# codelion/adaptive-classifier

Measured on NVIDIA H100. Metric: queries/sec predict() bert-base 128-tok, 1M x 768 prototypes, higher is better.
Workload: dtype f16

## Files before the change

### adaptive_classifier_b200/csrc/common.cuh

```cuda
#pragma once

#include <cuda_runtime.h>
#include <cuda.h>
#include <stdint.h>
#include <stdio.h>
#include <string.h>
#include <string>

#include "../../include/adaptive_b200.h"

namespace ac {

void set_error(const char *fmt, ...);
int check_cuda(cudaError_t e, const char *what);

#define AC_CUDA(call)                                                \
    do {                                                             \
        int _rc = ::ac::check_cuda((call), #call);                   \
        if (_rc != 0) return _rc;                                    \
    } while (0)

#define AC_REQUIRE(cond, ...)                                        \
    do {                                                             \
        if (!(cond)) {                                               \
// ... 58 lines not shown
    uint32_t ok;
    asm volatile(
        "{\n\t"
        ".reg .pred p;\n\t"
        "mbarrier.try_wait.parity.shared::cta.b64 p, [%1], %2;\n\t"
        "selp.u32 %0, 1, 0, p;\n\t"
        "}"
        : "=r"(ok)
        : "r"(smem_u32(bar)), "r"(parity)
        : "memory");
    return ok != 0;
}
__device__ __forceinline__ void mbar_wait(uint64_t *bar, uint32_t parity) {
    while (!mbar_try_wait(bar, parity)) {
    }
}

__device__ __forceinline__ void tma_prefetch_desc(const CUtensorMap *m) {
    asm volatile("prefetch.tensormap [%0];" ::"l"(reinterpret_cast<uint64_t>(m)) : "memory");
}
__device__ __forceinline__ void tma_load_2d(void *smem_dst, const CUtensorMap *m, uint64_t *bar, int c0, int c1) {
    asm volatile(
        "cp.async.bulk.tensor.2d.shared::cluster.global.tile.mbarrier::complete_tx::bytes [%0], [%1, {%3, %4}], [%2];"
        ::"r"(smem_u32(smem_dst)), "l"(reinterpret_cast<uint64_t>(m)), "r"(smem_u32(bar)), "r"(c0), "r"(c1)
        : "memory");
}
__device__ __forceinline__ void fence_proxy_async_smem() {
    asm volatile("fence.proxy.async.shared::cta;" ::: "memory");
}

__device__ __forceinline__ void named_bar_sync(int id, int nthreads) {
    asm volatile("bar.sync %0, %1;" ::"r"(id), "r"(nthreads) : "memory");
}

__device__ __forceinline__ uint64_t wgmma_desc_sw128(uint32_t smem_addr) {
    uint64_t d = 0;
    d |= static_cast<uint64_t>((smem_addr & 0x3FFFFu) >> 4);
    d |= static_cast<uint64_t>(1) << 16;
    d |= static_cast<uint64_t>(1024 >> 4) << 32;
    d |= static_cast<uint64_t>(1) << 62;
    return d;
}
__device__ __forceinline__ void wgmma_fence() { asm volatile("wgmma.fence.sync.aligned;" ::: "memory"); }
__device__ __forceinline__ void wgmma_commit() { asm volatile("wgmma.commit_group.sync.aligned;" ::: "memory"); }
template <int N>
__device__ __forceinline__ void wgmma_wait() { asm volatile("wgmma.wait_group.sync.aligned %0;" ::"n"(N) : "memory"); }

__device__ __forceinline__ void wgmma_m64n128_f16(float (&d)[64], uint64_t a_desc, uint64_t b_desc, uint32_t accumulate) {
    asm volatile(
        "{\n\t"
        ".reg .pred p;\n\t"
        "setp.ne.b32 p, %66, 0;\n\t"
        "wgmma.mma_async.sync.aligned.m64n128k16.f32.f16.f16 "
        "{%0, %1, %2, %3, %4, %5, %6, %7, %8, %9, %10, %11, %12, %13, %14, %15, "
        "%16, %17, %18, %19, %20, %21, %22, %23, %24, %25, %26, %27, %28, %29, %30, %31, "
        "%32, %33, %34, %35, %36, %37, %38, %39, %40, %41, %42, %43, %44, %45, %46, %47, "
        "%48, %49, %50, %51, %52, %53, %54, %55, %56, %57, %58, %59, %60, %61, %62, %63}, "
        "%64, %65, p, 1, 1, 0, 0;\n\t"
        "}"
        : "+f"(d[0]), "+f"(d[1]), "+f"(d[2]), "+f"(d[3]), "+f"(d[4]), "+f"(d[5]), "+f"(d[6]), "+f"(d[7]),
          "+f"(d[8]), "+f"(d[9]), "+f"(d[10]), "+f"(d[11]), "+f"(d[12]), "+f"(d[13]), "+f"(d[14]), "+f"(d[15]),
          "+f"(d[16]), "+f"(d[17]), "+f"(d[18]), "+f"(d[19]), "+f"(d[20]), "+f"(d[21]), "+f"(d[22]), "+f"(d[23]),
          "+f"(d[24]), "+f"(d[25]), "+f"(d[26]), "+f"(d[27]), "+f"(d[28]), "+f"(d[29]), "+f"(d[30]), "+f"(d[31]),
          "+f"(d[32]), "+f"(d[33]), "+f"(d[34]), "+f"(d[35]), "+f"(d[36]), "+f"(d[37]), "+f"(d[38]), "+f"(d[39]),
          "+f"(d[40]), "+f"(d[41]), "+f"(d[42]), "+f"(d[43]), "+f"(d[44]), "+f"(d[45]), "+f"(d[46]), "+f"(d[47]),
          "+f"(d[48]), "+f"(d[49]), "+f"(d[50]), "+f"(d[51]), "+f"(d[52]), "+f"(d[53]), "+f"(d[54]), "+f"(d[55]),
          "+f"(d[56]), "+f"(d[57]), "+f"(d[58]), "+f"(d[59]), "+f"(d[60]), "+f"(d[61]), "+f"(d[62]), "+f"(d[63])
// ... 77 lines not shown
```

### adaptive_classifier_b200/csrc/encoder.cu

```cuda
#include "gemm_tc.cuh"
#include <cuda_fp16.h>
#include <math_constants.h>
#include <algorithm>
#include <vector>

namespace ac {

__device__ __forceinline__ float ex2_approx(float x) {
    float y;
    asm("ex2.approx.ftz.f32 %0, %1;" : "=f"(y) : "f"(x));
    return y;
}
__device__ __forceinline__ float rcp_approx(float x) {
    float y;
    asm("rcp.approx.ftz.f32 %0, %1;" : "=f"(y) : "f"(x));
    return y;
}
__device__ __forceinline__ float gelu_erf(float y) {
    const float ay = fabsf(y);
    const float t = rcp_approx(fmaf(0.3275911f * 0.70710678118654752440f, ay, 1.f));
    float p = fmaf(0.5f * 1.061405429f, t, 0.5f * -1.453152027f);
    p = fmaf(p, t, 0.5f * 1.421413741f);
    p = fmaf(p, t, 0.5f * -0.284496736f);
    p = fmaf(p, t, 0.5f * 0.254829592f);
    const float e = ex2_approx((y * y) * (-0.5f * 1.4426950408889634f));
    const float h = (p * t) * e;
    return fmaxf(y, 0.f) - fabsf(y * h);
}

template <int MODE, bool OUT_HALF, bool VT, bool DEFER = false, bool ROPE = false>
struct EpiLinear {
    static_assert(!DEFER || (OUT_HALF && MODE != 2), "the deferred-LayerNorm consumer epilogues write fp16 operands");
    static_assert((MODE != 3 && !ROPE) || OUT_HALF, "the GeGLU / RoPE epilogues write fp16 operands");
    const float *__restrict__ bias;
    const float *__restrict__ residual;
    void *Y;
    int M, N, ldy;
    int round_out;
    __half *vT;
    int vt_col0, S, S_pad, H;
    const float *__restrict__ c1;
    const float2 *__restrict__ row_stats;
    const float *__restrict__ rope;

    static constexpr int kUnrollChunks = 4;
    static constexpr int kPrefetchDist = 1;
    struct State {
        float4 res[(MODE == 2) ? 2 : 1][(MODE == 2) ? 8 : 1];
        float mu, r;
    };
    __device__ __forceinline__ float pre(const State &st, float acc, float b, float c1v) const {
        return DEFER ? fmaf(st.r, fmaf(-st.mu, c1v, acc), b) : acc + b;
    }
    __device__ __forceinline__ bool skip_kernel() const { return false; }
    __device__ __forceinline__ void begin_cta(State &, int, int) const {}
    __device__ __forceinline__ void end_cta(State &, int, int) const {}

    __device__ __forceinline__ float act(float y) const {
        if (MODE == 1) y = gelu_erf(y);
        return y;
    }

    __device__ __forceinline__ void prefetch(State &st, const GemmTileInfo &ti, int row, int col0, int lane, int buf) const {
        if (DEFER) {
            if (((col0 - ti.n0) & (GEMM_EPI_COLS - 1)) == 0) {
                const float2 ms = (row < M) ? __ldg(row_stats + row) : make_float2(0.f, 0.f);
                st.mu = ms.x;
                st.r = ms.y;
            }
        }
        if (MODE != 2) return;
        const int row_base = row - lane;
        const int r8 = lane >> 2, c = lane & 3;
#pragma unroll
        for (int half = 0; half < 2; ++half) {
            const int col = col0 + 16 * half + 4 * c;
#pragma unroll
            for (int i = 0; i < 4; ++i) {
                const int grow = row_base + r8 + 8 * i;
                st.res[buf][half * 4 + i] =
                    (grow < M && col + 4 <= N)
                        ? __ldg(reinterpret_cast<const float4 *>(residual + static_cast<int64_t>(grow) * ldy + col))
                        : make_float4(0, 0, 0, 0);
            }
        }
    }

    __device__ __forceinline__ void tile(State &st, const GemmTileInfo &ti, int row, int col0, const float (&v)[32],
                                         uint8_t *stage, int lane, int buf, const float *acc) const {
// ... 103 lines not shown
                        const float4 a = *reinterpret_cast<const float4 *>(stage + rr * GEMM_EPI_STAGE_ROW_BYTES + 16 * c);
                        float4 o;
                        o.x = act(a.x + b4.x); o.y = act(a.y + b4.y); o.z = act(a.z + b4.z); o.w = act(a.w + b4.w);
                        if (MODE == 2) {
                            const float4 rs = st.res[buf][half * 4 + i];
                            o.x += rs.x; o.y += rs.y; o.z += rs.z; o.w += rs.w;
                        }
                        if (round_out) { o.x = round_tf32(o.x); o.y = round_tf32(o.y); o.z = round_tf32(o.z); o.w = round_tf32(o.w); }
                        *reinterpret_cast<float4 *>(Yf + static_cast<int64_t>(grow) * ldy + col) = o;
                    }
                }
                __syncwarp();
            }
        }
    }
};

struct EpiResidDefer {
    const float *__restrict__ bias;
    float *y;
    __half *yh;
    const float2 *__restrict__ stats_prev;
    const float *__restrict__ gamma;
    const float *__restrict__ beta;
    float2 *parts;
    int64_t part_stride;
    int M, N, ld;

    static constexpr int kUnrollChunks = 4;
#ifndef AC_RESID_PREFETCH
#define AC_RESID_PREFETCH 1
#endif
    static constexpr int kPrefetchDist = AC_RESID_PREFETCH;
    struct State {
        float4 res[kPrefetchDist + 1][8];
        float2 ms[4];
        float sum[4], sq[4];
    };
    __device__ __forceinline__ bool skip_kernel() const { return false; }
    __device__ __forceinline__ void begin_cta(State &, int, int) const {}
    __device__ __forceinline__ void end_cta(State &, int, int) const {}

    __device__ __forceinline__ void prefetch(State &st, const GemmTileInfo &ti, int row, int col0, int lane, int buf) const {
        const int row_base = row - lane;
        const int r8 = lane >> 2, c = lane & 3;
        if (((col0 - ti.n0) & (GEMM_EPI_COLS - 1)) == 0) {
#pragma unroll
            for (int i = 0; i < 4; ++i) {
                const int grow = row_base + r8 + 8 * i;
                st.ms[i] = (grow < M) ? __ldg(stats_prev + grow) : make_float2(0.f, 0.f);
                st.sum[i] = 0.f;
                st.sq[i] = 0.f;
            }
        }
#pragma unroll
        for (int half = 0; half < 2; ++half) {
            const int col = col0 + 16 * half + 4 * c;
#pragma unroll
            for (int i = 0; i < 4; ++i) {
                const int grow = row_base + r8 + 8 * i;
                st.res[buf][half * 4 + i] = (grow < M && col + 4 <= N)
                                                ? *reinterpret_cast<const float4 *>(y + static_cast<int64_t>(grow) * ld + col)
                                                : make_float4(0, 0, 0, 0);
            }
        }
    }

    __device__ __forceinline__ void tile(State &st, const GemmTileInfo &ti, int row, int col0, const float (&v)[32], uint8_t *stage,
                                         int lane, int buf, const float *) const {
        const int row_base = row - lane;
        if (row_base >= M || col0 >= N) return;
        const int r8 = lane >> 2, c = lane & 3;
#pragma unroll
        for (int half = 0; half < 2; ++half) {
            const int col = col0 + 16 * half + 4 * c;
            float4 *srow = reinterpret_cast<float4 *>(stage + lane * GEMM_EPI_STAGE_ROW_BYTES);
#pragma unroll
            for (int j = 0; j < 4; ++j)
                srow[j] = make_float4(v[16 * half + 4 * j], v[16 * half + 4 * j + 1], v[16 * half + 4 * j + 2], v[16 * half + 4 * j + 3]);
            __syncwarp();
            const bool col_ok = col + 4 <= N;
            const float4 b4 = col_ok ? __ldg(reinterpret_cast<const float4 *>(bias + col)) : make_float4(0, 0, 0, 0);
            const float4 g4 = col_ok ? __ldg(reinterpret_cast<const float4 *>(gamma + col)) : make_float4(0, 0, 0, 0);
            const float4 e4 = col_ok ? __ldg(reinterpret_cast<const float4 *>(beta + col)) : make_float4(0, 0, 0, 0);
#pragma unroll
            for (int i = 0; i < 4; ++i) {
                const int rr = r8 + 8 * i;
                const int grow = row_base + rr;
                if (grow < M && col_ok) {
                    const float4 a = *reinterpret_cast<const float4 *>(stage + rr * GEMM_EPI_STAGE_ROW_BYTES + 16 * c);
                    const float4 rs = st.res[buf][half * 4 + i];
                    const float mu = st.ms[i].x, r = st.ms[i].y;
                    float4 o;
                    o.x = (a.x + b4.x) + fmaf((rs.x - mu) * r, g4.x, e4.x);
                    o.y = (a.y + b4.y) + fmaf((rs.y - mu) * r, g4.y, e4.y);
                    o.z = (a.z + b4.z) + fmaf((rs.z - mu) * r, g4.z, e4.z);
                    o.w = (a.w + b4.w) + fmaf((rs.w - mu) * r, g4.w, e4.w);
                    *reinterpret_cast<float4 *>(y + static_cast<int64_t>(grow) * ld + col) = o;
                    const __half2 h0 = __floats2half2_rn(o.x, o.y), h1 = __floats2half2_rn(o.z, o.w);
                    uint2 pk;
                    pk.x = *reinterpret_cast<const uint32_t *>(&h0);
                    pk.y = *reinterpret_cast<const uint32_t *>(&h1);
                    *reinterpret_cast<uint2 *>(yh + static_cast<int64_t>(grow) * ld + col) = pk;
                    st.sum[i] += (o.x + o.y) + (o.z + o.w);
                    st.sq[i] += (o.x * o.x + o.y * o.y) + (o.z * o.z + o.w * o.w);
                }
            }
            __syncwarp();
        }
        if (((col0 - ti.n0) & (GEMM_EPI_COLS - 1)) == GEMM_EPI_COLS - 32) {
            const int part = col0 / GEMM_EPI_COLS;
#pragma unroll
            for (int i = 0; i < 4; ++i) {
                float s = st.sum[i], q = st.sq[i];
                s += __shfl_xor_sync(0xffffffffu, s, 1);
                q += __shfl_xor_sync(0xffffffffu, q, 1);
                s += __shfl_xor_sync(0xffffffffu, s, 2);
                q += __shfl_xor_sync(0xffffffffu, q, 2);
                const int grow = row_base + r8 + 8 * i;
                if (c == 0 && grow < M) parts[static_cast<int64_t>(part) * part_stride + grow] = make_float2(s, q);
            }
        }
    }
};

// ... 1064 lines not shown
```

### adaptive_classifier_b200/csrc/gemm_tc.cuh

```cuda
#pragma once
#include "common.cuh"

namespace ac {

constexpr int GEMM_BLOCK_M = 128;
constexpr int GEMM_BLOCK_N = 128;
constexpr int GEMM_BLOCK_K = 32;
constexpr int GEMM_KIND_TF32 = 0, GEMM_KIND_F16 = 1;
__host__ __device__ constexpr int gemm_block_k(int kind) { return kind == GEMM_KIND_F16 ? 64 : 32; }
constexpr int GEMM_STAGES = 4;
constexpr int GEMM_EPI_COLS = GEMM_BLOCK_N / 2;
constexpr int GEMM_EPI_WARPS = 8;
constexpr int GEMM_PRODUCER_THREAD = 32 * GEMM_EPI_WARPS;
constexpr int GEMM_THREADS = 32 * GEMM_EPI_WARPS + 128;
constexpr int GEMM_A_STAGE_BYTES = GEMM_BLOCK_M * 128;
constexpr int GEMM_B_STAGE_BYTES = GEMM_BLOCK_N * 128;
constexpr int GEMM_STAGE_BYTES = GEMM_A_STAGE_BYTES + GEMM_B_STAGE_BYTES;
constexpr int GEMM_ACC_LD = GEMM_BLOCK_N + 4;
constexpr int GEMM_ACC_BYTES = GEMM_BLOCK_M * GEMM_ACC_LD * 4;
constexpr int GEMM_EPI_STAGE_ROW_BYTES = 80;
constexpr int GEMM_EPI_STAGE_BYTES = 32 * GEMM_EPI_STAGE_ROW_BYTES;
constexpr int GEMM_SMEM_BYTES = GEMM_STAGES * GEMM_STAGE_BYTES + GEMM_ACC_BYTES + GEMM_EPI_WARPS * GEMM_EPI_STAGE_BYTES +
                                1024  + 256 ;
static_assert(GEMM_SMEM_BYTES <= 227 * 1024, "stage ring + accumulator tile do not fit");

#ifndef AC_MBAR_WATCHDOG
#define AC_MBAR_WATCHDOG 1
#endif

__device__ __forceinline__ void mbar_wait_guarded(uint64_t *bar, uint32_t parity) {
#if AC_MBAR_WATCHDOG
    uint32_t spins = 0;
    while (!mbar_try_wait(bar, parity)) {
        if (++spins > (1u << 26)) __trap();
    }
#else
    mbar_wait(bar, parity);
#endif
}

struct GemmTileInfo {
    int m0, n0;
    int tile_iter;
};

__device__ __forceinline__ int gemm_epi_chalf() { return ((threadIdx.x >> 5) >> 1) & 1; }

template <class Epi, bool kMFastest = false, int kKind = GEMM_KIND_TF32>
__global__ void __launch_bounds__(GEMM_THREADS, 1)
gemm_tc_kernel(const __grid_constant__ CUtensorMap tmap_a, const __grid_constant__ CUtensorMap tmap_b,
               int M, int N, int K, Epi epi) {
    if (epi.skip_kernel()) return;
    extern __shared__ uint8_t smem_raw[];
    uint8_t *smem = reinterpret_cast<uint8_t *>((reinterpret_cast<uintptr_t>(smem_raw) + 1023) & ~uintptr_t(1023));
    uint8_t *smem_a = smem;
    uint8_t *smem_b = smem + GEMM_STAGES * GEMM_A_STAGE_BYTES;
    float *acc_tile = reinterpret_cast<float *>(smem + GEMM_STAGES * GEMM_STAGE_BYTES);
    uint8_t *epi_stage = smem + GEMM_STAGES * GEMM_STAGE_BYTES + GEMM_ACC_BYTES;
    uint64_t *bars = reinterpret_cast<uint64_t *>(epi_stage + GEMM_EPI_WARPS * GEMM_EPI_STAGE_BYTES);
    uint64_t *full_bar = bars;
    uint64_t *empty_bar = bars + GEMM_STAGES;

    const int warp = threadIdx.x >> 5;
    const int lane = threadIdx.x & 31;
    const int tiles_m = (M + GEMM_BLOCK_M - 1) / GEMM_BLOCK_M;
    const int tiles_n = (N + GEMM_BLOCK_N - 1) / GEMM_BLOCK_N;
    const int num_tiles = tiles_m * tiles_n;
    constexpr int BK = gemm_block_k(kKind);
    const int num_kb = (K + BK - 1) / BK;

    if (threadIdx.x == GEMM_PRODUCER_THREAD) {
        tma_prefetch_desc(&tmap_a);
        tma_prefetch_desc(&tmap_b);
        for (int s = 0; s < GEMM_STAGES; ++s) {
            mbar_init(&full_bar[s], 1);
            mbar_init(&empty_bar[s], GEMM_EPI_WARPS);
        }
        fence_mbar_init();
    }
    __syncthreads();

    if (threadIdx.x >= GEMM_PRODUCER_THREAD) {
        if (threadIdx.x == GEMM_PRODUCER_THREAD) {
            int stage = 0;
            uint32_t phase = 0;
            for (int tile = blockIdx.x; tile < num_tiles; tile += gridDim.x) {
                const int m0 = (kMFastest ? tile % tiles_m : tile / tiles_n) * GEMM_BLOCK_M;
                const int n0 = (kMFastest ? tile / tiles_m : tile % tiles_n) * GEMM_BLOCK_N;
                for (int kb = 0; kb < num_kb; ++kb) {
                    mbar_wait_guarded(&empty_bar[stage], phase ^ 1);
                    mbar_arrive_expect_tx(&full_bar[stage], GEMM_STAGE_BYTES);
                    tma_load_2d(smem_a + stage * GEMM_A_STAGE_BYTES, &tmap_a, &full_bar[stage], kb * BK, m0);
                    tma_load_2d(smem_b + stage * GEMM_B_STAGE_BYTES, &tmap_b, &full_bar[stage], kb * BK, n0);
                    if (++stage == GEMM_STAGES) { stage = 0; phase ^= 1; }
                }
            }
        }
        return;
    }

    const int wg = warp >> 2;
    const int q = 2 * wg + (warp & 1);
    const int chalf = gemm_epi_chalf();
    typename Epi::State est;
    epi.begin_cta(est, q, lane);
    int stage = 0;
    uint32_t phase = 0;
    int it = 0;
    const float *acc_row = acc_tile + (q * 32 + lane) * GEMM_ACC_LD;
    for (int tile = blockIdx.x; tile < num_tiles; tile += gridDim.x, ++it) {
        GemmTileInfo ti;
        ti.m0 = (kMFastest ? tile % tiles_m : tile / tiles_n) * GEMM_BLOCK_M;
        ti.n0 = (kMFastest ? tile / tiles_m : tile % tiles_n) * GEMM_BLOCK_N;
        ti.tile_iter = it;
        const int row = ti.m0 + q * 32 + lane;
        const int c_lo = chalf * GEMM_EPI_COLS;
        constexpr int kDist = Epi::kPrefetchDist, kBufs = kDist + 1, kChunks = GEMM_EPI_COLS / 32;
#pragma unroll
        for (int d = 0; d < kDist; ++d)
            if (d < kChunks) epi.prefetch(est, ti, row, ti.n0 + c_lo + 32 * d, lane, d % kBufs);

        float acc[64];
#pragma unroll
        for (int j = 0; j < 64; ++j) acc[j] = 0.f;
        int prev_stage = -1;
        for (int kb = 0; kb < num_kb; ++kb) {
            mbar_wait_guarded(&full_bar[stage], phase);
            const uint64_t a_desc = wgmma_desc_sw128(smem_u32(smem_a + stage * GEMM_A_STAGE_BYTES + wg * 64 * 128));
            const uint64_t b_desc = wgmma_desc_sw128(smem_u32(smem_b + stage * GEMM_B_STAGE_BYTES));
            wgmma_fence();
#pragma unroll
            for (int k = 0; k < 4; ++k) {
                if (kKind == GEMM_KIND_F16) wgmma_m64n128_f16(acc, a_desc + 2 * k, b_desc + 2 * k, 1u);
                else wgmma_m64n128_tf32(acc, a_desc + 2 * k, b_desc + 2 * k, 1u);
            }
            wgmma_commit();
            wgmma_wait<1>();
            __syncwarp();
            if (prev_stage >= 0 && lane == 0) mbar_arrive(&empty_bar[prev_stage]);
            prev_stage = stage;
            if (++stage == GEMM_STAGES) { stage = 0; phase ^= 1; }
        }
        wgmma_wait<0>();
        __syncwarp();
        if (lane == 0) mbar_arrive(&empty_bar[prev_stage]);

        named_bar_sync(1 + wg, 128);
        wgmma_store_acc(acc, acc_tile + wg * 64 * GEMM_ACC_LD, GEMM_ACC_LD);
        named_bar_sync(1 + wg, 128);
#pragma unroll (Epi::kUnrollChunks)
        for (int ci = 0; ci < kChunks; ++ci) {
            const int c = c_lo + 32 * ci;
            if (ci + kDist < kChunks) epi.prefetch(est, ti, row, ti.n0 + c + 32 * kDist, lane, (ci + kDist) % kBufs);
            float v[32];
            acc_row_ld32(acc_row + c, v);
            epi.tile(est, ti, row, ti.n0 + c, v, epi_stage + warp * GEMM_EPI_STAGE_BYTES, lane, ci % kBufs, acc_row + c);
        }
    }
    epi.end_cta(est, q, lane);
}

template <class Epi, bool kMFastest = false, int kKind = GEMM_KIND_TF32>
int launch_gemm_tc(const CUtensorMap &ta, const CUtensorMap &tb, int M, int N, int K, const Epi &epi,
                   cudaStream_t stream, int max_ctas = 0, int prof_cls = PROF_GEMM_LINEAR, double prof_bytes = 0.0) {
    auto kern = gemm_tc_kernel<Epi, kMFastest, kKind>;
    static bool attr_set[64] = {};
    int dev = 0;
    AC_CUDA(cudaGetDevice(&dev));
    if (dev < 0 || dev >= 64 || !attr_set[dev]) {
        AC_CUDA(cudaFuncSetAttribute(kern, cudaFuncAttributeMaxDynamicSharedMemorySize, GEMM_SMEM_BYTES));
        if (dev >= 0 && dev < 64) attr_set[dev] = true;
    }
    const int tiles = ((M + GEMM_BLOCK_M - 1) / GEMM_BLOCK_M) * ((N + GEMM_BLOCK_N - 1) / GEMM_BLOCK_N);
    int ctas = sm_count();
    if (max_ctas > 0 && max_ctas < ctas) ctas = max_ctas;
    if (tiles < ctas) ctas = tiles;
    if (ctas <= 0) return AC_OK;
    const int slot = prof_begin(prof_cls, 2.0 * M * static_cast<double>(N) * K, prof_bytes, stream);
    kern<<<ctas, GEMM_THREADS, GEMM_SMEM_BYTES, stream>>>(ta, tb, M, N, K, epi);
    prof_end(slot, stream);
    AC_LAUNCH_CHECK();
    return AC_OK;
}

}
```

### adaptive_classifier_b200/csrc/knn_tc.cu

```cuda
#include "gemm_tc.cuh"
#include <cuda_fp16.h>
#include <math_constants.h>

namespace ac {

int launch_knn_rerank(const float *Q, const float *P, int B, int64_t N, int D, int kc, const int32_t *cand, float *out_d,
                      int64_t *out_i, int64_t row_offset, cudaStream_t stream);
size_t topk_select_workspace(int B, int64_t L, int k);
int topk_select(const float *d, const int64_t *idx, int B, int64_t L, int64_t in_stride, int64_t id_offset, int k,
                float *out_d, int64_t *out_i, void *ws, size_t ws_bytes, cudaStream_t stream, const float *row_gate = nullptr);
int knn_exact_subset(const float *Q, const float *P, int B, int64_t N, int D, int k, float *out_d, int64_t *out_i,
                     int64_t row_offset, void *ws, size_t ws_bytes, cudaStream_t s);
size_t knn_exact_workspace_pub(int B, int64_t N, int k);

constexpr int KNN_KC = 16;
constexpr int KNN_KP = 32;

__device__ __forceinline__ uint32_t key_to_ord(float f) {
    const uint32_t u = __float_as_uint(f);
    return (u & 0x80000000u) ? ~u : (u | 0x80000000u);
}
__device__ __forceinline__ float ord_to_key(uint32_t o) {
    return __uint_as_float((o & 0x80000000u) ? (o & 0x7fffffffu) : ~o);
}

struct EpiKnn {
    const float *p_sqnorm;
    float *cand_key;
    int32_t *cand_idx;
    uint32_t *gthr;
    int B;
    int64_t N;
    int tiles_m, slots;
    int kt;

    static constexpr int kUnrollChunks = 1;
    static constexpr int kPrefetchDist = 1;
    struct State {
        float key[KNN_KC];
        int32_t idx[KNN_KC];
        float pn[2];
        float gt;
    };

    __device__ __forceinline__ bool skip_kernel() const { return false; }
    __device__ __forceinline__ void begin_cta(State &st, int, int) const {
#pragma unroll
        for (int i = 0; i < KNN_KC; ++i) { st.key[i] = CUDART_INF_F; st.idx[i] = -1; }
        st.pn[0] = st.pn[1] = CUDART_INF_F;
        st.gt = CUDART_INF_F;
    }

    __device__ __forceinline__ void prefetch(State &st, const GemmTileInfo &, int row, int col0, int lane, int buf) const {
        const int64_t n = static_cast<int64_t>(col0) + lane;
        const float x = (n < N) ? __ldg(p_sqnorm + n) : CUDART_INF_F;
        if (buf) st.pn[1] = x; else st.pn[0] = x;
        if (buf == 0) {
            float pub = CUDART_INF_F;
#pragma unroll
            for (int i = 0; i < KNN_KC; ++i) pub = (i == kt - 1) ? st.key[i] : pub;
            if (pub < CUDART_INF_F) atomicMin(gthr + row, key_to_ord(pub));
            st.gt = ord_to_key(*reinterpret_cast<volatile uint32_t *>(gthr + row));
        }
    }

    __device__ __forceinline__ void insert(State &st, float key, int32_t n) const {
#pragma unroll
        for (int i = KNN_KC - 1; i > 0; --i) {
            const bool shift = key < st.key[i - 1];
            const bool here = !shift && (key < st.key[i]);
            const float nk = shift ? st.key[i - 1] : (here ? key : st.key[i]);
            const int32_t ni = shift ? st.idx[i - 1] : (here ? n : st.idx[i]);
            st.key[i] = nk;
            st.idx[i] = ni;
        }
        if (key < st.key[0]) { st.key[0] = key; st.idx[0] = n; }
    }

    __device__ __forceinline__ void tile(State &st, const GemmTileInfo &, int , int col0, const float (&v)[32],
                                         uint8_t * , int , int buf, const float *acc) const {
        const float pn_lane = buf ? st.pn[1] : st.pn[0];
        const float thr = fminf(st.key[KNN_KC - 1], st.gt);
        uint32_t hits = 0;
#pragma unroll
        for (int j = 0; j < 32; ++j) {
            const float pn = __shfl_sync(0xffffffffu, pn_lane, j);
            const float key = fmaf(-2.f, v[j], pn);
            hits |= (key < thr) ? (1u << j) : 0u;
        }
        uint32_t uni = __reduce_or_sync(0xffffffffu, hits);
        while (uni) {
            const int j = __ffs(uni) - 1;
            uni &= uni - 1;
            const float key = fmaf(-2.f, acc[j], __shfl_sync(0xffffffffu, pn_lane, j));
            const int64_t n = static_cast<int64_t>(col0) + j;
            if (((hits >> j) & 1u) && key < fminf(st.key[KNN_KC - 1], st.gt) && n < N) insert(st, key, static_cast<int32_t>(n));
        }
    }

    __device__ __forceinline__ void end_cta(State &st, int q, int lane) const {
        const int chalf = gemm_epi_chalf();
        const int mt = blockIdx.x % tiles_m;
        const int slot = (blockIdx.x / tiles_m) * 2 + chalf;
        const int row = mt * GEMM_BLOCK_M + q * 32 + lane;
        if (row >= B) return;
        float *ck = cand_key + (static_cast<int64_t>(row) * slots + slot) * KNN_KC;
        int32_t *ci = cand_idx + (static_cast<int64_t>(row) * slots + slot) * KNN_KC;
#pragma unroll
        for (int i = 0; i < KNN_KC; ++i) { ck[i] = st.key[i]; ci[i] = st.idx[i]; }
    }
};

struct EpiKnnCollect {
    const float *p_sqnorm;
    const float *thr;
    int32_t *buf;
    int32_t *cnt;
    const int32_t *need;
    int cap, B;
    int64_t N;
    int tiles_m;

    static constexpr int kUnrollChunks = 1;
    static constexpr int kPrefetchDist = 1;
    struct State {
        float pn[2];
        float thr;
    };
    __device__ __forceinline__ bool skip_kernel() const { return *reinterpret_cast<const volatile int32_t *>(need) == 0; }
    __device__ __forceinline__ void begin_cta(State &st, int q, int lane) const {
        const int row = (blockIdx.x % tiles_m) * GEMM_BLOCK_M + q * 32 + lane;
        st.thr = (row < B) ? thr[row] : -CUDART_INF_F;
        st.pn[0] = st.pn[1] = CUDART_INF_F;
    }
    __device__ __forceinline__ void prefetch(State &st, const GemmTileInfo &, int, int col0, int lane, int buf_) const {
        const int64_t n = static_cast<int64_t>(col0) + lane;
        const float x = (n < N) ? __ldg(p_sqnorm + n) : CUDART_INF_F;
        if (buf_) st.pn[1] = x; else st.pn[0] = x;
    }
    __device__ __forceinline__ void tile(State &st, const GemmTileInfo &, int row, int col0, const float (&v)[32], uint8_t *,
                                         int, int buf_, const float *) const {
        const float pn_lane = buf_ ? st.pn[1] : st.pn[0];
        uint32_t hits = 0;
#pragma unroll
        for (int j = 0; j < 32; ++j) {
            const float pn = __shfl_sync(0xffffffffu, pn_lane, j);
            const float key = fmaf(-2.f, v[j], pn);
            hits |= (key <= st.thr) ? (1u << j) : 0u;
        }
        while (hits) {
            const int j = __ffs(hits) - 1;
            hits &= hits - 1;
            const int64_t n = static_cast<int64_t>(col0) + j;
            if (n < N) {
                const int pos = atomicAdd(cnt + row, 1);
                if (pos < cap) buf[static_cast<int64_t>(row) * cap + pos] = static_cast<int32_t>(n);
            }
        }
    }
    __device__ __forceinline__ void end_cta(State &, int, int) const {}
};


__global__ void knn_prep_queries_kernel(const float *__restrict__ Q, int B, int D, float *__restrict__ Qr,
                                        __half *__restrict__ Qh, float *__restrict__ qn) {
    const int row = blockIdx.x * (blockDim.x >> 5) + (threadIdx.x >> 5);
    const int lane = threadIdx.x & 31;
    if (row >= B) return;
    float s = 0.f;
    for (int i = lane; i < D; i += 32) {
        const float x = Q[static_cast<int64_t>(row) * D + i];
        if (Qh) Qh[static_cast<int64_t>(row) * D + i] = __float2half_rn(x);
        else Qr[static_cast<int64_t>(row) * D + i] = round_tf32(x);
        s = fmaf(x, x, s);
    }
    s = warp_sum(s);
    if (lane == 0) qn[row] = s;
}

__global__ void knn_prep_rows_kernel(const float *__restrict__ P, int64_t N, int D, float *__restrict__ pn) {
    const int64_t row = static_cast<int64_t>(blockIdx.x) * 8 + (threadIdx.x >> 5);
    const int lane = threadIdx.x & 31;
    if (row >= N) return;
    const float *p = P + row * D;
    float s = 0.f;
    for (int i = lane; i < D; i += 32) s = fmaf(p[i], p[i], s);
    s = warp_sum(s);
    if (lane == 0) pn[row] = s;
}

__global__ void knn_max_norm_kernel(const float *__restrict__ pn, int64_t N, float *__restrict__ out) {
    float m = 0.f;
    const int64_t stride = static_cast<int64_t>(gridDim.x) * blockDim.x;
// ... 343 lines not shown
```

Measured before the change: 12160.

## Add ping-pong warpgroup scheduling to persistent GEMM for encoder epilogues

Adds a ping-pong mode to the persistent TMA/wgmma GEMM. The two consumer warpgroups take alternate tiles, each computing a full 128x128 tile with two m64 wgmma chains, and named barriers hand off the MMA turn and the shared accumulator buffer, so one group's epilogue overlaps the other's mainloop. Register budgets are rebalanced with setmaxnreg (producer decreased, consumers increased). It is enabled for encoder linear epilogues except GELU/GeGLU, and for the residual-LayerNorm epilogue. KNN scans keep the cooperative path. The risks are register pressure from the doubled accumulators and barrier ordering hazards.

```diff
diff --git a/adaptive_classifier_b200/csrc/common.cuh b/adaptive_classifier_b200/csrc/common.cuh
--- a/adaptive_classifier_b200/csrc/common.cuh
+++ b/adaptive_classifier_b200/csrc/common.cuh
@@ -114,6 +114,13 @@
 __device__ __forceinline__ void named_bar_sync(int id, int nthreads) {
     asm volatile("bar.sync %0, %1;" ::"r"(id), "r"(nthreads) : "memory");
 }
+__device__ __forceinline__ void named_bar_arrive(int id, int nthreads) {
+    asm volatile("bar.arrive %0, %1;" ::"r"(id), "r"(nthreads) : "memory");
+}
+template <int N>
+__device__ __forceinline__ void setmaxnreg_inc() { asm volatile("setmaxnreg.inc.sync.aligned.u32 %0;" ::"n"(N)); }
+template <int N>
+__device__ __forceinline__ void setmaxnreg_dec() { asm volatile("setmaxnreg.dec.sync.aligned.u32 %0;" ::"n"(N)); }
 
 __device__ __forceinline__ uint64_t wgmma_desc_sw128(uint32_t smem_addr) {
     uint64_t d = 0;
diff --git a/adaptive_classifier_b200/csrc/encoder.cu b/adaptive_classifier_b200/csrc/encoder.cu
--- a/adaptive_classifier_b200/csrc/encoder.cu
+++ b/adaptive_classifier_b200/csrc/encoder.cu
@@ -45,6 +45,7 @@
 
     static constexpr int kUnrollChunks = 4;
     static constexpr int kPrefetchDist = 1;
+    static constexpr bool kPingPong = MODE != 1 && MODE != 3;
     struct State {
         float4 res[(MODE == 2) ? 2 : 1][(MODE == 2) ? 8 : 1];
         float mu, r;
@@ -53,8 +54,8 @@
         return DEFER ? fmaf(st.r, fmaf(-st.mu, c1v, acc), b) : acc + b;
     }
     __device__ __forceinline__ bool skip_kernel() const { return false; }
-    __device__ __forceinline__ void begin_cta(State &, int, int) const {}
-    __device__ __forceinline__ void end_cta(State &, int, int) const {}
+    __device__ __forceinline__ void begin_cta(State &, int, int, int) const {}
+    __device__ __forceinline__ void end_cta(State &, int, int, int) const {}
 
     __device__ __forceinline__ float act(float y) const {
         if (MODE == 1) y = gelu_erf(y);
@@ -224,14 +225,15 @@
 #define AC_RESID_PREFETCH 1
 #endif
     static constexpr int kPrefetchDist = AC_RESID_PREFETCH;
+    static constexpr bool kPingPong = true;
     struct State {
         float4 res[kPrefetchDist + 1][8];
         float2 ms[4];
         float sum[4], sq[4];
     };
     __device__ __forceinline__ bool skip_kernel() const { return false; }
-    __device__ __forceinline__ void begin_cta(State &, int, int) const {}
-    __device__ __forceinline__ void end_cta(State &, int, int) const {}
+    __device__ __forceinline__ void begin_cta(State &, int, int, int) const {}
+    __device__ __forceinline__ void end_cta(State &, int, int, int) const {}
 
     __device__ __forceinline__ void prefetch(State &st, const GemmTileInfo &ti, int row, int col0, int lane, int buf) const {
         const int row_base = row - lane;
@@ -241,8 +243,6 @@
             for (int i = 0; i < 4; ++i) {
                 const int grow = row_base + r8 + 8 * i;
                 st.ms[i] = (grow < M) ? __ldg(stats_prev + grow) : make_float2(0.f, 0.f);
-                st.sum[i] = 0.f;
-                st.sq[i] = 0.f;
             }
         }
 #pragma unroll
@@ -263,6 +263,10 @@
         const int row_base = row - lane;
         if (row_base >= M || col0 >= N) return;
         const int r8 = lane >> 2, c = lane & 3;
+        if (((col0 - ti.n0) & (GEMM_EPI_COLS - 1)) == 0) {
+#pragma unroll
+            for (int i = 0; i < 4; ++i) { st.sum[i] = 0.f; st.sq[i] = 0.f; }
+        }
 #pragma unroll
         for (int half = 0; half < 2; ++half) {
             const int col = col0 + 16 * half + 4 * c;
diff --git a/adaptive_classifier_b200/csrc/gemm_tc.cuh b/adaptive_classifier_b200/csrc/gemm_tc.cuh
--- a/adaptive_classifier_b200/csrc/gemm_tc.cuh
+++ b/adaptive_classifier_b200/csrc/gemm_tc.cuh
@@ -13,6 +13,8 @@
 constexpr int GEMM_EPI_WARPS = 8;
 constexpr int GEMM_PRODUCER_THREAD = 32 * GEMM_EPI_WARPS;
 constexpr int GEMM_THREADS = 32 * GEMM_EPI_WARPS + 128;
+constexpr int GEMM_PRODUCER_REGS = 24, GEMM_CONSUMER_REGS = 240;
+constexpr int GEMM_BAR_WG = 1, GEMM_BAR_ACC_FREE = 3, GEMM_BAR_MMA_TURN = 5;
 constexpr int GEMM_A_STAGE_BYTES = GEMM_BLOCK_M * 128;
 constexpr int GEMM_B_STAGE_BYTES = GEMM_BLOCK_N * 128;
 constexpr int GEMM_STAGE_BYTES = GEMM_A_STAGE_BYTES + GEMM_B_STAGE_BYTES;
@@ -44,12 +46,87 @@
     int tile_iter;
 };
 
-__device__ __forceinline__ int gemm_epi_chalf() { return ((threadIdx.x >> 5) >> 1) & 1; }
+
+template <int kKind, int kHalves>
+__device__ __forceinline__ void gemm_mainloop(float (&acc)[kHalves][64], const uint8_t *smem_a, const uint8_t *smem_b, int a_off,
+                                              uint64_t *full_bar, uint64_t *empty_bar, int kb0, int num_kb, int lane,
+                                              int turn_bar) {
+#pragma unroll
+    for (int h = 0; h < kHalves; ++h)
+#pragma unroll
+        for (int j = 0; j < 64; ++j) acc[h][j] = 0.f;
+    int prev_stage = -1;
+    for (int kb = 0; kb < num_kb; ++kb) {
+        const int g = kb0 + kb;
+        const int stage = g % GEMM_STAGES;
+        mbar_wait_guarded(&full_bar[stage], static_cast<uint32_t>(g / GEMM_STAGES) & 1u);
+        if (kb == num_kb - 1 && turn_bar >= 0) named_bar_arrive(turn_bar, 256);
+        const uint64_t a_desc = wgmma_desc_sw128(smem_u32(smem_a + stage * GEMM_A_STAGE_BYTES + a_off));
+        const uint64_t b_desc = wgmma_desc_sw128(smem_u32(smem_b + stage * GEMM_B_STAGE_BYTES));
+        wgmma_fence();
+#pragma unroll
+        for (int k = 0; k < 4; ++k) {
+#pragma unroll
+            for (int h = 0; h < kHalves; ++h) {
+                if (kKind == GEMM_KIND_F16) wgmma_m64n128_f16(acc[h], a_desc + 512 * h + 2 * k, b_desc + 2 * k, 1u);
+                else wgmma_m64n128_tf32(acc[h], a_desc + 512 * h + 2 * k, b_desc + 2 * k, 1u);
+            }
+        }
+        wgmma_commit();
+        wgmma_wait<1>();
+        __syncwarp();
+        if (prev_stage >= 0 && lane == 0) mbar_arrive(&empty_bar[prev_stage]);
+        prev_stage = stage;
+    }
+    wgmma_wait<0>();
+    __syncwarp();
+    if (lane == 0) mbar_arrive(&empty_bar[prev_stage]);
+}
+
+template <class Epi, int kChunks>
+__device__ __forceinline__ void gemm_epi_prefetch_head(const Epi &epi, typename Epi::State &est, const GemmTileInfo &ti, int row,
+                                                       int c_lo, int lane) {
+    constexpr int kDist = Epi::kPrefetchDist, kBufs = kDist + 1;
+#pragma unroll
+    for (int d = 0; d < kDist; ++d)
+        if (d < kChunks) epi.prefetch(est, ti, row, ti.n0 + c_lo + 32 * d, lane, d % kBufs);
+}
+
+template <class Epi, int kChunks>
+__device__ __forceinline__ void gemm_epi_drain(const Epi &epi, typename Epi::State &est, const GemmTileInfo &ti,
+                                               const float *acc_row, int row, int c_lo, uint8_t *stage, int lane) {
+    constexpr int kDist = Epi::kPrefetchDist, kBufs = kDist + 1;
+#pragma unroll (Epi::kUnrollChunks)
+    for (int ci = 0; ci < kChunks; ++ci) {
+        const int c = c_lo + 32 * ci;
+        if (ci + kDist < kChunks) epi.prefetch(est, ti, row, ti.n0 + c + 32 * kDist, lane, (ci + kDist) % kBufs);
+        float v[32];
+        acc_row_ld32(acc_row + c, v);
+        epi.tile(est, ti, row, ti.n0 + c, v, stage, lane, ci % kBufs, acc_row + c);
+    }
+}
+
+template <bool kMFastest, int kKind>
+struct GemmGrid {
+    int tiles_m, tiles_n, num_tiles, num_kb;
+    __device__ __forceinline__ GemmGrid(int M, int N, int K)
+        : tiles_m((M + GEMM_BLOCK_M - 1) / GEMM_BLOCK_M), tiles_n((N + GEMM_BLOCK_N - 1) / GEMM_BLOCK_N),
+          num_tiles(tiles_m * tiles_n), num_kb((K + gemm_block_k(kKind) - 1) / gemm_block_k(kKind)) {}
+    __device__ __forceinline__ GemmTileInfo tile(int t, int it) const {
+        GemmTileInfo ti;
+        ti.m0 = (kMFastest ? t % tiles_m : t / tiles_n) * GEMM_BLOCK_M;
+        ti.n0 = (kMFastest ? t / tiles_m : t % tiles_n) * GEMM_BLOCK_N;
+        ti.tile_iter = it;
+        return ti;
+    }
+};
 
 template <class Epi, bool kMFastest = false, int kKind = GEMM_KIND_TF32>
 __global__ void __launch_bounds__(GEMM_THREADS, 1)
 gemm_tc_kernel(const __grid_constant__ CUtensorMap tmap_a, const __grid_constant__ CUtensorMap tmap_b,
                int M, int N, int K, Epi epi) {
+    constexpr bool kPingPong = Epi::kPingPong;
+    static_assert(!(kPingPong && kMFastest), "the m-fastest scans keep per-(query, CTA, column half) state: cooperative only");
     if (epi.skip_kernel()) return;
     extern __shared__ uint8_t smem_raw[];
     uint8_t *smem = reinterpret_cast<uint8_t *>((reinterpret_cast<uintptr_t>(smem_raw) + 1023) & ~uintptr_t(1023));
@@ -63,35 +140,32 @@
 
     const int warp = threadIdx.x >> 5;
     const int lane = threadIdx.x & 31;
-    const int tiles_m = (M + GEMM_BLOCK_M - 1) / GEMM_BLOCK_M;
-    const int tiles_n = (N + GEMM_BLOCK_N - 1) / GEMM_BLOCK_N;
-    const int num_tiles = tiles_m * tiles_n;
     constexpr int BK = gemm_block_k(kKind);
-    const int num_kb = (K + BK - 1) / BK;
 
     if (threadIdx.x == GEMM_PRODUCER_THREAD) {
         tma_prefetch_desc(&tmap_a);
         tma_prefetch_desc(&tmap_b);
         for (int s = 0; s < GEMM_STAGES; ++s) {
             mbar_init(&full_bar[s], 1);
-            mbar_init(&empty_bar[s], GEMM_EPI_WARPS);
+            mbar_init(&empty_bar[s], kPingPong ? 4 : GEMM_EPI_WARPS);
         }
         fence_mbar_init();
     }
     __syncthreads();
 
     if (threadIdx.x >= GEMM_PRODUCER_THREAD) {
+        if constexpr (kPingPong) setmaxnreg_dec<GEMM_PRODUCER_REGS>();
         if (threadIdx.x == GEMM_PRODUCER_THREAD) {
+            const GemmGrid<kMFastest, kKind> grid(M, N, K);
             int stage = 0;
             uint32_t phase = 0;
-            for (int tile = blockIdx.x; tile < num_tiles; tile += gridDim.x) {
-                const int m0 = (kMFastest ? tile % tiles_m : tile / tiles_n) * GEMM_BLOCK_M;
-                const int n0 = (kMFastest ? tile / tiles_m : tile % tiles_n) * GEMM_BLOCK_N;
-                for (int kb = 0; kb < num_kb; ++kb) {
+            for (int tile = blockIdx.x; tile < grid.num_tiles; tile += gridDim.x) {
+                const GemmTileInfo ti = grid.tile(tile, 0);
+                for (int kb = 0; kb < grid.num_kb; ++kb) {
                     mbar_wait_guarded(&empty_bar[stage], phase ^ 1);
                     mbar_arrive_expect_tx(&full_bar[stage], GEMM_STAGE_BYTES);
-                    tma_load_2d(smem_a + stage * GEMM_A_STAGE_BYTES, &tmap_a, &full_bar[stage], kb * BK, m0);
-                    tma_load_2d(smem_b + stage * GEMM_B_STAGE_BYTES, &tmap_b, &full_bar[stage], kb * BK, n0);
+                    tma_load_2d(smem_a + stage * GEMM_A_STAGE_BYTES, &tmap_a, &full_bar[stage], kb * BK, ti.m0);
+                    tma_load_2d(smem_b + stage * GEMM_B_STAGE_BYTES, &tmap_b, &full_bar[stage], kb * BK, ti.n0);
                     if (++stage == GEMM_STAGES) { stage = 0; phase ^= 1; }
                 }
             }
@@ -100,64 +174,54 @@
     }
 
     const int wg = warp >> 2;
-    const int q = 2 * wg + (warp & 1);
-    const int chalf = gemm_epi_chalf();
     typename Epi::State est;
-    epi.begin_cta(est, q, lane);
-    int stage = 0;
-    uint32_t phase = 0;
-    int it = 0;
-    const float *acc_row = acc_tile + (q * 32 + lane) * GEMM_ACC_LD;
-    for (int tile = blockIdx.x; tile < num_tiles; tile += gridDim.x, ++it) {
-        GemmTileInfo ti;
-        ti.m0 = (kMFastest ? tile % tiles_m : tile / tiles_n) * GEMM_BLOCK_M;
-        ti.n0 = (kMFastest ? tile / tiles_m : tile % tiles_n) * GEMM_BLOCK_N;
-        ti.tile_iter = it;
-        const int row = ti.m0 + q * 32 + lane;
-        const int c_lo = chalf * GEMM_EPI_COLS;
-        constexpr int kDist = Epi::kPrefetchDist, kBufs = kDist + 1, kChunks = GEMM_EPI_COLS / 32;
-#pragma unroll
-        for (int d = 0; d < kDist; ++d)
-            if (d < kChunks) epi.prefetch(est, ti, row, ti.n0 + c_lo + 32 * d, lane, d % kBufs);
-
-        float acc[64];
-#pragma unroll
-        for (int j = 0; j < 64; ++j) acc[j] = 0.f;
-        int prev_stage = -1;
-        for (int kb = 0; kb < num_kb; ++kb) {
-            mbar_wait_guarded(&full_bar[stage], phase);
-            const uint64_t a_desc = wgmma_desc_sw128(smem_u32(smem_a + stage * GEMM_A_STAGE_BYTES + wg * 64 * 128));
-            const uint64_t b_desc = wgmma_desc_sw128(smem_u32(smem_b + stage * GEMM_B_STAGE_BYTES));
-            wgmma_fence();
-#pragma unroll
-            for (int k = 0; k < 4; ++k) {
-                if (kKind == GEMM_KIND_F16) wgmma_m64n128_f16(acc, a_desc + 2 * k, b_desc + 2 * k, 1u);
-                else wgmma_m64n128_tf32(acc, a_desc + 2 * k, b_desc + 2 * k, 1u);
-            }
-            wgmma_commit();
-            wgmma_wait<1>();
-            __syncwarp();
-            if (prev_stage >= 0 && lane == 0) mbar_arrive(&empty_bar[prev_stage]);
-            prev_stage = stage;
-            if (++stage == GEMM_STAGES) { stage = 0; phase ^= 1; }
-        }
-        wgmma_wait<0>();
-        __syncwarp();
-        if (lane == 0) mbar_arrive(&empty_bar[prev_stage]);
-
-        named_bar_sync(1 + wg, 128);
-        wgmma_store_acc(acc, acc_tile + wg * 64 * GEMM_ACC_LD, GEMM_ACC_LD);
-        named_bar_sync(1 + wg, 128);
-#pragma unroll (Epi::kUnrollChunks)
-        for (int ci = 0; ci < kChunks; ++ci) {
-            const int c = c_lo + 32 * ci;
-            if (ci + kDist < kChunks) epi.prefetch(est, ti, row, ti.n0 + c + 32 * kDist, lane, (ci + kDist) % kBufs);
-            float v[32];
-            acc_row_ld32(acc_row + c, v);
-            epi.tile(est, ti, row, ti.n0 + c, v, epi_stage + warp * GEMM_EPI_STAGE_BYTES, lane, ci % kBufs, acc_row + c);
-        }
-    }
-    epi.end_cta(est, q, lane);
+    if constexpr (kPingPong) {
+        setmaxnreg_inc<GEMM_CONSUMER_REGS>();
+        const GemmGrid<kMFastest, kKind> grid(M, N, K);
+        const int q = warp & 3;
+        const float *acc_row = acc_tile + (q * 32 + lane) * GEMM_ACC_LD;
+        uint8_t *stage = epi_stage + warp * GEMM_EPI_STAGE_BYTES;
+        epi.begin_cta(est, q, -1, lane);
+        for (int it = wg;; it += 2) {
+            const int tile = blockIdx.x + it * gridDim.x;
+            if (tile >= grid.num_tiles) break;
+            const GemmTileInfo ti = grid.tile(tile, it);
+            const int row = ti.m0 + q * 32 + lane;
+            const bool next = tile + static_cast<int>(gridDim.x) < grid.num_tiles;
+            gemm_epi_prefetch_head<Epi, GEMM_BLOCK_N / 32>(epi, est, ti, row, 0, lane);
+            float acc[2][64];
+            if (it > 0) named_bar_sync(GEMM_BAR_MMA_TURN + wg, 256);
+            gemm_mainloop<kKind, 2>(acc, smem_a, smem_b, 0, full_bar, empty_bar, it * grid.num_kb, grid.num_kb, lane,
+                                    next ? GEMM_BAR_MMA_TURN + (wg ^ 1) : -1);
+            if (it > 0) named_bar_sync(GEMM_BAR_ACC_FREE + wg, 256);
+            wgmma_store_acc(acc[0], acc_tile, GEMM_ACC_LD);
+            wgmma_store_acc(acc[1], acc_tile + 64 * GEMM_ACC_LD, GEMM_ACC_LD);
+            named_bar_sync(GEMM_BAR_WG + wg, 128);
+            gemm_epi_drain<Epi, GEMM_BLOCK_N / 32>(epi, est, ti, acc_row, row, 0, stage, lane);
+            if (next) named_bar_arrive(GEMM_BAR_ACC_FREE + (wg ^ 1), 256);
+        }
+        epi.end_cta(est, q, -1, lane);
+    } else {
+        const GemmGrid<kMFastest, kKind> grid(M, N, K);
+        const int q = 2 * wg + (warp & 1);
+        const int chalf = (warp >> 1) & 1;
+        const float *acc_row = acc_tile + (q * 32 + lane) * GEMM_ACC_LD;
+        uint8_t *stage = epi_stage + warp * GEMM_EPI_STAGE_BYTES;
+        epi.begin_cta(est, q, chalf, lane);
+        int it = 0;
+        for (int tile = blockIdx.x; tile < grid.num_tiles; tile += gridDim.x, ++it) {
+            const GemmTileInfo ti = grid.tile(tile, it);
+            const int row = ti.m0 + q * 32 + lane;
+            gemm_epi_prefetch_head<Epi, GEMM_EPI_COLS / 32>(epi, est, ti, row, chalf * GEMM_EPI_COLS, lane);
+            float acc[1][64];
+            gemm_mainloop<kKind, 1>(acc, smem_a, smem_b, wg * 64 * 128, full_bar, empty_bar, it * grid.num_kb, grid.num_kb, lane, -1);
+            named_bar_sync(GEMM_BAR_WG + wg, 128);
+            wgmma_store_acc(acc[0], acc_tile + wg * 64 * GEMM_ACC_LD, GEMM_ACC_LD);
+            named_bar_sync(GEMM_BAR_WG + wg, 128);
+            gemm_epi_drain<Epi, GEMM_EPI_COLS / 32>(epi, est, ti, acc_row, row, chalf * GEMM_EPI_COLS, stage, lane);
+        }
+        epi.end_cta(est, q, chalf, lane);
+    }
 }
 
 template <class Epi, bool kMFastest = false, int kKind = GEMM_KIND_TF32>
diff --git a/adaptive_classifier_b200/csrc/knn_tc.cu b/adaptive_classifier_b200/csrc/knn_tc.cu
--- a/adaptive_classifier_b200/csrc/knn_tc.cu
+++ b/adaptive_classifier_b200/csrc/knn_tc.cu
@@ -36,6 +36,7 @@
 
     static constexpr int kUnrollChunks = 1;
     static constexpr int kPrefetchDist = 1;
+    static constexpr bool kPingPong = false;
     struct State {
         float key[KNN_KC];
         int32_t idx[KNN_KC];
@@ -44,7 +45,7 @@
     };
 
     __device__ __forceinline__ bool skip_kernel() const { return false; }
-    __device__ __forceinline__ void begin_cta(State &st, int, int) const {
+    __device__ __forceinline__ void begin_cta(State &st, int, int, int) const {
 #pragma unroll
         for (int i = 0; i < KNN_KC; ++i) { st.key[i] = CUDART_INF_F; st.idx[i] = -1; }
         st.pn[0] = st.pn[1] = CUDART_INF_F;
@@ -98,8 +99,7 @@
         }
     }
 
-    __device__ __forceinline__ void end_cta(State &st, int q, int lane) const {
-        const int chalf = gemm_epi_chalf();
+    __device__ __forceinline__ void end_cta(State &st, int q, int chalf, int lane) const {
         const int mt = blockIdx.x % tiles_m;
         const int slot = (blockIdx.x / tiles_m) * 2 + chalf;
         const int row = mt * GEMM_BLOCK_M + q * 32 + lane;
@@ -123,12 +123,13 @@
 
     static constexpr int kUnrollChunks = 1;
     static constexpr int kPrefetchDist = 1;
+    static constexpr bool kPingPong = false;
     struct State {
         float pn[2];
         float thr;
     };
     __device__ __forceinline__ bool skip_kernel() const { return *reinterpret_cast<const volatile int32_t *>(need) == 0; }
-    __device__ __forceinline__ void begin_cta(State &st, int q, int lane) const {
+    __device__ __forceinline__ void begin_cta(State &st, int q, int, int lane) const {
         const int row = (blockIdx.x % tiles_m) * GEMM_BLOCK_M + q * 32 + lane;
         st.thr = (row < B) ? thr[row] : -CUDART_INF_F;
         st.pn[0] = st.pn[1] = CUDART_INF_F;
@@ -158,7 +159,7 @@
             }
         }
     }
-    __device__ __forceinline__ void end_cta(State &, int, int) const {}
+    __device__ __forceinline__ void end_cta(State &, int, int, int) const {}
 };
 
 
```

After: 12370 (median of 6 runs). 1.02x the previous value.

## Split GEMM into dedicated MMA warpgroup and epilogue warps with register rebalancing

Applied to the files above, without the earlier changes.

Adds a dedicated MMA warpgroup that computes both 64-row halves of each tile into two accumulators and hands results to the epilogue warps through acc_full/acc_empty mbarriers. The epilogue of tile i can then overlap with the MMA for tile i+1, instead of the same warps doing MMA and epilogue in sequence. setmaxnreg moves registers from the producer to the MMA and epilogue warps, and epilogue prefetch state is trimmed (stats loaded per row, MODE 2 prefetch disabled) to fit 160 registers. The single acc_tile buffer still serialises MMA stores against the epilogue, and the block grows to 512 threads.

```diff
diff --git a/adaptive_classifier_b200/csrc/common.cuh b/adaptive_classifier_b200/csrc/common.cuh
--- a/adaptive_classifier_b200/csrc/common.cuh
+++ b/adaptive_classifier_b200/csrc/common.cuh
@@ -115,6 +115,11 @@
     asm volatile("bar.sync %0, %1;" ::"r"(id), "r"(nthreads) : "memory");
 }
 
+template <int N>
+__device__ __forceinline__ void setmaxnreg_inc() { asm volatile("setmaxnreg.inc.sync.aligned.u32 %0;" ::"n"(N)); }
+template <int N>
+__device__ __forceinline__ void setmaxnreg_dec() { asm volatile("setmaxnreg.dec.sync.aligned.u32 %0;" ::"n"(N)); }
+
 __device__ __forceinline__ uint64_t wgmma_desc_sw128(uint32_t smem_addr) {
     uint64_t d = 0;
     d |= static_cast<uint64_t>((smem_addr & 0x3FFFFu) >> 4);
diff --git a/adaptive_classifier_b200/csrc/encoder.cu b/adaptive_classifier_b200/csrc/encoder.cu
--- a/adaptive_classifier_b200/csrc/encoder.cu
+++ b/adaptive_classifier_b200/csrc/encoder.cu
@@ -44,9 +44,9 @@
     const float *__restrict__ rope;
 
     static constexpr int kUnrollChunks = 4;
-    static constexpr int kPrefetchDist = 1;
+    static constexpr int kPrefetchDist = (MODE == 2) ? 0 : 1;
     struct State {
-        float4 res[(MODE == 2) ? 2 : 1][(MODE == 2) ? 8 : 1];
+        float4 res[1][(MODE == 2) ? 8 : 1];
         float mu, r;
     };
     __device__ __forceinline__ float pre(const State &st, float acc, float b, float c1v) const {
@@ -226,7 +226,6 @@
     static constexpr int kPrefetchDist = AC_RESID_PREFETCH;
     struct State {
         float4 res[kPrefetchDist + 1][8];
-        float2 ms[4];
         float sum[4], sq[4];
     };
     __device__ __forceinline__ bool skip_kernel() const { return false; }
@@ -239,8 +238,6 @@
         if (((col0 - ti.n0) & (GEMM_EPI_COLS - 1)) == 0) {
 #pragma unroll
             for (int i = 0; i < 4; ++i) {
-                const int grow = row_base + r8 + 8 * i;
-                st.ms[i] = (grow < M) ? __ldg(stats_prev + grow) : make_float2(0.f, 0.f);
                 st.sum[i] = 0.f;
                 st.sq[i] = 0.f;
             }
@@ -282,7 +279,8 @@
                 if (grow < M && col_ok) {
                     const float4 a = *reinterpret_cast<const float4 *>(stage + rr * GEMM_EPI_STAGE_ROW_BYTES + 16 * c);
                     const float4 rs = st.res[buf][half * 4 + i];
-                    const float mu = st.ms[i].x, r = st.ms[i].y;
+                    const float2 ms = __ldg(stats_prev + grow);
+                    const float mu = ms.x, r = ms.y;
                     float4 o;
                     o.x = (a.x + b4.x) + fmaf((rs.x - mu) * r, g4.x, e4.x);
                     o.y = (a.y + b4.y) + fmaf((rs.y - mu) * r, g4.y, e4.y);
diff --git a/adaptive_classifier_b200/csrc/gemm_tc.cuh b/adaptive_classifier_b200/csrc/gemm_tc.cuh
--- a/adaptive_classifier_b200/csrc/gemm_tc.cuh
+++ b/adaptive_classifier_b200/csrc/gemm_tc.cuh
@@ -11,8 +11,11 @@
 constexpr int GEMM_STAGES = 4;
 constexpr int GEMM_EPI_COLS = GEMM_BLOCK_N / 2;
 constexpr int GEMM_EPI_WARPS = 8;
-constexpr int GEMM_PRODUCER_THREAD = 32 * GEMM_EPI_WARPS;
-constexpr int GEMM_THREADS = 32 * GEMM_EPI_WARPS + 128;
+constexpr int GEMM_MMA_THREAD0 = 32 * GEMM_EPI_WARPS;
+constexpr int GEMM_PRODUCER_THREAD = GEMM_MMA_THREAD0 + 128;
+constexpr int GEMM_THREADS = GEMM_PRODUCER_THREAD + 128;
+constexpr int GEMM_EPI_REGS = 160, GEMM_MMA_REGS = 160, GEMM_PRODUCER_REGS = 24;
+static_assert(128 * GEMM_PRODUCER_REGS + 128 * GEMM_MMA_REGS + 256 * GEMM_EPI_REGS <= 65536, "register split exceeds the file");
 constexpr int GEMM_A_STAGE_BYTES = GEMM_BLOCK_M * 128;
 constexpr int GEMM_B_STAGE_BYTES = GEMM_BLOCK_N * 128;
 constexpr int GEMM_STAGE_BYTES = GEMM_A_STAGE_BYTES + GEMM_B_STAGE_BYTES;
@@ -60,6 +63,8 @@
     uint64_t *bars = reinterpret_cast<uint64_t *>(epi_stage + GEMM_EPI_WARPS * GEMM_EPI_STAGE_BYTES);
     uint64_t *full_bar = bars;
     uint64_t *empty_bar = bars + GEMM_STAGES;
+    uint64_t *acc_full = bars + 2 * GEMM_STAGES;
+    uint64_t *acc_empty = acc_full + 1;
 
     const int warp = threadIdx.x >> 5;
     const int lane = threadIdx.x & 31;
@@ -68,19 +73,23 @@
     const int num_tiles = tiles_m * tiles_n;
     constexpr int BK = gemm_block_k(kKind);
     const int num_kb = (K + BK - 1) / BK;
+    const int my_tiles = (num_tiles - static_cast<int>(blockIdx.x) + static_cast<int>(gridDim.x) - 1) / static_cast<int>(gridDim.x);
 
     if (threadIdx.x == GEMM_PRODUCER_THREAD) {
         tma_prefetch_desc(&tmap_a);
         tma_prefetch_desc(&tmap_b);
         for (int s = 0; s < GEMM_STAGES; ++s) {
             mbar_init(&full_bar[s], 1);
-            mbar_init(&empty_bar[s], GEMM_EPI_WARPS);
-        }
+            mbar_init(&empty_bar[s], 4);
+        }
+        mbar_init(acc_full, 128);
+        mbar_init(acc_empty, 32 * GEMM_EPI_WARPS);
         fence_mbar_init();
     }
     __syncthreads();
 
     if (threadIdx.x >= GEMM_PRODUCER_THREAD) {
+        setmaxnreg_dec<GEMM_PRODUCER_REGS>();
         if (threadIdx.x == GEMM_PRODUCER_THREAD) {
             int stage = 0;
             uint32_t phase = 0;
@@ -99,16 +108,60 @@
         return;
     }
 
+    if (threadIdx.x >= GEMM_MMA_THREAD0) {
+        setmaxnreg_inc<GEMM_MMA_REGS>();
+        const uint64_t a_desc0 = wgmma_desc_sw128(smem_u32(smem_a));
+        const uint64_t b_desc0 = wgmma_desc_sw128(smem_u32(smem_b));
+        int stage = 0;
+        uint32_t phase = 0;
+        for (int it = 0; it < my_tiles; ++it) {
+            float acc0[64], acc1[64];
+#pragma unroll
+            for (int j = 0; j < 64; ++j) { acc0[j] = 0.f; acc1[j] = 0.f; }
+            int prev_stage = -1;
+            for (int kb = 0; kb < num_kb; ++kb) {
+                mbar_wait_guarded(&full_bar[stage], phase);
+                const uint64_t a_desc = a_desc0 + stage * (GEMM_A_STAGE_BYTES >> 4);
+                const uint64_t b_desc = b_desc0 + stage * (GEMM_B_STAGE_BYTES >> 4);
+                wgmma_fence();
+#pragma unroll
+                for (int k = 0; k < 4; ++k) {
+                    if (kKind == GEMM_KIND_F16) {
+                        wgmma_m64n128_f16(acc0, a_desc + 2 * k, b_desc + 2 * k, 1u);
+                        wgmma_m64n128_f16(acc1, a_desc + 512 + 2 * k, b_desc + 2 * k, 1u);
+                    } else {
+                        wgmma_m64n128_tf32(acc0, a_desc + 2 * k, b_desc + 2 * k, 1u);
+                        wgmma_m64n128_tf32(acc1, a_desc + 512 + 2 * k, b_desc + 2 * k, 1u);
+                    }
+                }
+                wgmma_commit();
+                wgmma_wait<1>();
+                __syncwarp();
+                if (prev_stage >= 0 && lane == 0) mbar_arrive(&empty_bar[prev_stage]);
+                prev_stage = stage;
+                if (++stage == GEMM_STAGES) { stage = 0; phase ^= 1; }
+            }
+            wgmma_wait<0>();
+            __syncwarp();
+            if (lane == 0) mbar_arrive(&empty_bar[prev_stage]);
+
+            mbar_wait_guarded(acc_empty, (it & 1) ^ 1);
+            wgmma_store_acc(acc0, acc_tile, GEMM_ACC_LD);
+            wgmma_store_acc(acc1, acc_tile + 64 * GEMM_ACC_LD, GEMM_ACC_LD);
+            mbar_arrive(acc_full);
+        }
+        return;
+    }
+
+    setmaxnreg_inc<GEMM_EPI_REGS>();
     const int wg = warp >> 2;
     const int q = 2 * wg + (warp & 1);
     const int chalf = gemm_epi_chalf();
     typename Epi::State est;
     epi.begin_cta(est, q, lane);
-    int stage = 0;
-    uint32_t phase = 0;
-    int it = 0;
     const float *acc_row = acc_tile + (q * 32 + lane) * GEMM_ACC_LD;
-    for (int tile = blockIdx.x; tile < num_tiles; tile += gridDim.x, ++it) {
+    for (int it = 0; it < my_tiles; ++it) {
+        const int tile = static_cast<int>(blockIdx.x) + it * static_cast<int>(gridDim.x);
         GemmTileInfo ti;
         ti.m0 = (kMFastest ? tile % tiles_m : tile / tiles_n) * GEMM_BLOCK_M;
         ti.n0 = (kMFastest ? tile / tiles_m : tile % tiles_n) * GEMM_BLOCK_N;
@@ -120,34 +173,7 @@
         for (int d = 0; d < kDist; ++d)
             if (d < kChunks) epi.prefetch(est, ti, row, ti.n0 + c_lo + 32 * d, lane, d % kBufs);
 
-        float acc[64];
-#pragma unroll
-        for (int j = 0; j < 64; ++j) acc[j] = 0.f;
-        int prev_stage = -1;
-        for (int kb = 0; kb < num_kb; ++kb) {
-            mbar_wait_guarded(&full_bar[stage], phase);
-            const uint64_t a_desc = wgmma_desc_sw128(smem_u32(smem_a + stage * GEMM_A_STAGE_BYTES + wg * 64 * 128));
-            const uint64_t b_desc = wgmma_desc_sw128(smem_u32(smem_b + stage * GEMM_B_STAGE_BYTES));
-            wgmma_fence();
-#pragma unroll
-            for (int k = 0; k < 4; ++k) {
-                if (kKind == GEMM_KIND_F16) wgmma_m64n128_f16(acc, a_desc + 2 * k, b_desc + 2 * k, 1u);
-                else wgmma_m64n128_tf32(acc, a_desc + 2 * k, b_desc + 2 * k, 1u);
-            }
-            wgmma_commit();
-            wgmma_wait<1>();
-            __syncwarp();
-            if (prev_stage >= 0 && lane == 0) mbar_arrive(&empty_bar[prev_stage]);
-            prev_stage = stage;
-            if (++stage == GEMM_STAGES) { stage = 0; phase ^= 1; }
-        }
-        wgmma_wait<0>();
-        __syncwarp();
-        if (lane == 0) mbar_arrive(&empty_bar[prev_stage]);
-
-        named_bar_sync(1 + wg, 128);
-        wgmma_store_acc(acc, acc_tile + wg * 64 * GEMM_ACC_LD, GEMM_ACC_LD);
-        named_bar_sync(1 + wg, 128);
+        mbar_wait_guarded(acc_full, it & 1);
 #pragma unroll (Epi::kUnrollChunks)
         for (int ci = 0; ci < kChunks; ++ci) {
             const int c = c_lo + 32 * ci;
@@ -156,6 +182,7 @@
             acc_row_ld32(acc_row + c, v);
             epi.tile(est, ti, row, ti.n0 + c, v, epi_stage + warp * GEMM_EPI_STAGE_BYTES, lane, ci % kBufs, acc_row + c);
         }
+        mbar_arrive(acc_empty);
     }
     epi.end_cta(est, q, lane);
 }
```

New measurement: 15950 before, 18000 after (median of 6 runs). +12.9%, better.
